# Leo-Liao-Chao/Uncertainty-Aware-CILQR-for-Trajectory-Optimization

Measured on AMD Instinct MI355X. Metric: CILQR solves/sec (N=50, batch B), higher is better.
Workload: dtype f64

## Files before the change

include/cilqr.h:

```cpp
#ifndef CILQR_H_
#define CILQR_H_

#include <stddef.h>
#include <stdint.h>

#ifdef __cplusplus
extern "C" {
#endif

#define CILQR_NX 4
#define CILQR_NU 2
#define CILQR_POLY_COEFFS 6
#define CILQR_MAX_HORIZON 384
#define CILQR_ABI_VERSION 2
#define CILQR_COMM_ID_BYTES 128
#define CILQR_MAX_POLYGONS 1024
#define CILQR_MAX_POLYGON_VERTICES 16

typedef struct cilqr_params {
  int32_t num_of_local_wpts;
  int32_t poly_order;
  int32_t horizon;
  int32_t max_iterations;
  int32_t num_states;
// ... 107 lines not shown
                                int32_t* iters_out, int32_t* status_out, uint32_t flags);
int cilqr_solve_batch_obstacles_device(cilqr_handle* h, void* stream, int B, int N, int M, const double* x0, double* U,
                                       const double* poly, const double* xplan_fl, const cilqr_obstacles* obs, double* X_out,
                                       double* J_out, int32_t* iters_out, int32_t* status_out, uint32_t flags);

int cilqr_set_uncertainty_map_device(cilqr_handle* h, const cilqr_uncertainty_map* map);
int cilqr_set_uncertainty_map(cilqr_handle* h, const cilqr_uncertainty_map* map);
int cilqr_clear_uncertainty_map(cilqr_handle* h);

int cilqr_debug_uncertainty_cost(cilqr_handle* h, int n, const double* states, double* cost, double* vx, double* mx);

int cilqr_solve_batch_sampled(cilqr_handle* h, int B, int N, int n_obs, int n_samples,
                              const double* x0, double* U, const double* poly, const double* xplan_fl,
                              const double* nom_pose, const double* nom_dim, const double* sample_offset,
                              double sample_weight, double* X_out, double* J_out, int32_t* iters_out,
                              int32_t* status_out, uint32_t flags);
int cilqr_solve_batch_sampled_device(cilqr_handle* h, void* stream, int B, int N, int n_obs, int n_samples,
                                     const double* x0, double* U, const double* poly, const double* xplan_fl,
                                     const double* nom_pose, const double* nom_dim, const double* sample_offset,
                                     double sample_weight, double* X_out, double* J_out, int32_t* iters_out,
                                     int32_t* status_out, uint32_t flags);

int cilqr_argmin_device(cilqr_handle* h, void* stream, int B, const double* J, double* out_pair);

#define CILQR_SCORE_FIELDS 8
typedef enum cilqr_score_field {
  CILQR_SCORE_TRACK = 0,
  CILQR_SCORE_CONTROL = 1,
  CILQR_SCORE_OBSTACLE = 2,
  CILQR_SCORE_UNCERTAINTY = 3,
  CILQR_SCORE_MAX_C = 4,
  CILQR_SCORE_MAX_C_ENTRY = 5,
  CILQR_SCORE_MAX_CTRL = 6,
  CILQR_SCORE_COLLISION = 7
} cilqr_score_field;
int cilqr_score_batch_device(cilqr_handle* h, void* stream, int B, int N, int M, const double* X, const double* U, const double* poly,
                             const double* xplan_fl, const cilqr_obstacles* obs, double max_collision, double* score, double* total);
int cilqr_score_batch(cilqr_handle* h, int B, int N, int M, const double* X, const double* U, const double* poly,
                      const double* xplan_fl, const cilqr_obstacles* obs, double max_collision, double* score, double* total);
int cilqr_score_batch_sampled_device(cilqr_handle* h, void* stream, int B, int N, int n_obs, int n_samples, const double* X,
                                     const double* U, const double* poly, const double* xplan_fl, const double* nom_pose,
                                     const double* nom_dim, const double* sample_offset, double sample_weight, double max_collision,
                                     double* score, double* total);
int cilqr_score_batch_sampled(cilqr_handle* h, int B, int N, int n_obs, int n_samples, const double* X, const double* U,
                              const double* poly, const double* xplan_fl, const double* nom_pose, const double* nom_dim,
                              const double* sample_offset, double sample_weight, double max_collision, double* score, double* total);
// ... 196 lines not shown
                              double max_risk, const double* base, double* risk, double* step_risk, double* pair_p, double* entry_p,
                              double* total);

int cilqr_predict_obstacles_device(cilqr_handle* h, void* stream, int T, int N, int M, const double* track, const double* track_dim,
                                   const double* track_cov, const double* track_noise, double* pose_out, double* dim_out,
                                   double* cov_out, double* sigma_out);
int cilqr_predict_obstacles(cilqr_handle* h, int T, int N, int M, const double* track, const double* track_dim, const double* track_cov,
                            const double* track_noise, double* pose_out, double* dim_out, double* cov_out, double* sigma_out);

int cilqr_chance_risk_cov_device(cilqr_handle* h, void* stream, int B, int N, int M, const double* X, const double* U, const double* K,
                                 const double* sigma0, int64_t sigma0_batch_stride, const double* process_noise,
                                 const cilqr_obstacles* obs, const double* obs_cov, uint32_t flags, double max_risk, const double* base,
                                 double* risk, double* step_risk, double* entry_p, double* sigma_out, double* total);
int cilqr_chance_risk_cov(cilqr_handle* h, int B, int N, int M, const double* X, const double* U, const double* K, const double* sigma0,
                          int64_t sigma0_batch_stride, const double* process_noise, const cilqr_obstacles* obs, const double* obs_cov,
                          uint32_t flags, double max_risk, const double* base, double* risk, double* step_risk, double* entry_p,
                          double* sigma_out, double* total);

int cilqr_comm_unique_id(void* id_bytes );
int cilqr_comm_init_rank(cilqr_handle* h, int n_ranks, int rank, const void* id_bytes);
int cilqr_comm_destroy(cilqr_handle* h);
int cilqr_comm_size(const cilqr_handle* h);
int cilqr_argmin_global_device(cilqr_handle* h, void* stream, int B, const double* J, int64_t index_offset, double* out_pair);

int cilqr_debug_select(cilqr_handle* h, int n, const double* triples, double* out_pair);

typedef struct cilqr_multi cilqr_multi;
int cilqr_create_multi(const cilqr_params* p, int max_batch_per_device, int max_horizon, int max_obstacles, int n_devices,
                       const int* devices, cilqr_multi** out);
int cilqr_multi_destroy(cilqr_multi* m);
int cilqr_multi_device_count(const cilqr_multi* m);
cilqr_handle* cilqr_multi_handle(cilqr_multi* m, int i);
int cilqr_shard_range(int B, int n_shards, int shard, int* first, int* count);
int cilqr_multi_solve_batch(cilqr_multi* m, int B, int N, int M, const double* x0, double* U, const double* poly,
                            const double* xplan_fl, const double* obs_pose, const double* obs_dim, const double* obs_weight,
                            double* X_out, double* J_out, int32_t* iters_out, int32_t* status_out, uint32_t flags,
                            int64_t* best_index, double* best_J);
int cilqr_multi_uses_rccl(const cilqr_multi* m);
int cilqr_debug_fail_enqueue(cilqr_handle* h, int nth_call);

int cilqr_set_diag_buffer(cilqr_handle* h, uint64_t* dev_buf);

int cilqr_set_pass_count_buffer(cilqr_handle* h, int32_t* dev_buf);

int cilqr_solve_family(const cilqr_handle* h, int B, int N, int M);
int cilqr_solve_wavefronts(const cilqr_handle* h, int B, int N, int M);
// ... 232 lines not shown
```

uncertainty-aware-cilqr-for-trajectory-optimization_amd/cilqr_amd/__init__.py:

```python
import ctypes as C
import os

import numpy as np

PKG_ROOT = os.path.dirname(os.path.dirname(os.path.abspath(__file__)))
LIB_PATH = os.environ.get("CILQR_LIB") or os.path.join(PKG_ROOT, "lib", "libcilqr_hip.so")

NX, NU, POLY = 4, 2, 6
FLAG_FAITHFUL_ITERS = 1
FLAG_GENERAL_ONLY = 2
EXIT_TOLERANCE, EXIT_LAMBDA_MAX, EXIT_MAX_ITER, EXIT_NUMERIC = 0, 1, 2, 3
SCORE_FIELDS = 8
(SCORE_TRACK, SCORE_CONTROL, SCORE_OBSTACLE, SCORE_UNCERTAINTY, SCORE_MAX_C, SCORE_MAX_C_ENTRY, SCORE_MAX_CTRL,
 SCORE_COLLISION) = range(SCORE_FIELDS)
RISK_FIELDS = 4
RISK_COLLISION, RISK_WORST_C, RISK_WORST_ROW, RISK_MEAN_TOTAL = range(RISK_FIELDS)
ROLLOUT_RISK_FIELDS = 6
RR_COLLISION, RR_WORST_C, RR_WORST_ROW, RR_WORST_ENTRY, RR_FIRST_STEP, RR_STEP_SHARE = range(ROLLOUT_RISK_FIELDS)
RRS_FIELDS = 8
(RRS_COLLISION, RRS_WORST_C, RRS_WORST_ROW, RRS_WORST_ENTRY, RRS_FIRST_STEP, RRS_STEP_SHARE, RRS_ANY_SHARE,
 RRS_PAIR_SHARE) = range(RRS_FIELDS)
MAP_RISK_FIELDS = 7
MR_COLLISION, MR_WORST_OCC, MR_WORST_ROW, MR_WORST_ENTRY, MR_FIRST_STEP, MR_STEP_SHARE, MR_UNKNOWN = range(MAP_RISK_FIELDS)
MAP_RISK_UNKNOWN_HITS = 1
# ... 35 lines not shown
TS_X, TS_Y, TS_VX, TS_VY, TS_P = 0, 1, 2, 3, 4
TS_SIZE_X, TS_SIZE_Y, TS_YAW, TS_ID, TS_HITS, TS_MISSES, TS_AGE, TS_DET = range(20, 28)
TRACK_WORLD_FIELDS = 9
(TW_NEXT_ID, TW_TICKS, TW_LIVE, TW_CONFIRMED, TW_MATCHED, TW_BORN, TW_DIED, TW_DROPPED,
 TW_INVALID) = range(TRACK_WORLD_FIELDS)
TRACK_RESET = 1
CLEAR_MOVERS_FIELDS = 8
(CM_MOVERS, CM_CLEARED, CM_OWNED_LINKED, CM_OWNED_HALO, CM_MAX_VALUE, CM_MAX_CELL, CM_CONTESTED,
 CM_KEPT_UNKNOWN) = range(CLEAR_MOVERS_FIELDS)
CLEAR_MOVERS_MAX_HALO2 = 1024
MAP_CLEARANCE_FIELDS = 8
(MC_CLEARANCE, MC_STEP, MC_CELL, MC_BELOW_STEPS, MC_FIRST_BELOW, MC_TOUCH_STEPS, MC_OFF_MAP_STEPS,
 MC_LOST_STEPS) = range(MAP_CLEARANCE_FIELDS)
MAP_CLEARANCE_UNKNOWN_SEEDS = 1
STOP_FIELDS = 8
(SP_STOP_STEP, SP_DISTANCE, SP_END_SPEED, SP_DEVIATION, SP_DEVIATION_STEP, SP_CLAMPED_STEPS, SP_OVERRUN_STEPS,
 SP_LOST) = range(STOP_FIELDS)
STOP_ALLOW_MOVING = 1
STOP_MIN_ADVANCE = 1.0e-3

ABI_SYMBOLS = (
    "cilqr_params_default", "cilqr_abi_version", "cilqr_device_count", "cilqr_last_error", "cilqr_default_control_seq",
    "cilqr_local_plan", "cilqr_local_plan_batch", "cilqr_local_plan_batch_device", "cilqr_create", "cilqr_destroy", "cilqr_host_alloc", "cilqr_host_free", "cilqr_solve_batch", "cilqr_solve_batch_device", "cilqr_solve_batch_obstacles", "cilqr_solve_batch_obstacles_device", "cilqr_solve_batch_sampled", "cilqr_solve_batch_sampled_device",
    "cilqr_argmin_device", "cilqr_wait", "cilqr_set_diag_buffer", "cilqr_set_pass_count_buffer", "cilqr_solve_family", "cilqr_solve_wavefronts", "cilqr_solve_sampled_wavefronts", "cilqr_debug_quu_inverse", "cilqr_debug_closest_sample", "cilqr_debug_blur_ellipse", "cilqr_warp_costmap", "cilqr_warp_costmap_device", "cilqr_warp_costmap_batch_device", "cilqr_blur_costmap", "cilqr_blur_costmap_device", "cilqr_blur_costmap_batch_device", "cilqr_map_geom_set",
    "cilqr_occupancy_to_layer", "cilqr_occupancy_to_layer_device", "cilqr_layer_to_occupancy", "cilqr_layer_to_occupancy_device",
    "cilqr_costmap_frame_device", "cilqr_costmap_frame_batch_device",
    "cilqr_boxes_to_polygons", "cilqr_rasterize_polygons", "cilqr_rasterize_polygons_device", "cilqr_warp_costmap_polygons_device",
    "cilqr_costmap_frame_polygons_device",
    "cilqr_set_uncertainty_map", "cilqr_set_uncertainty_map_device", "cilqr_clear_uncertainty_map", "cilqr_debug_uncertainty_cost",
    "cilqr_comm_unique_id", "cilqr_comm_init_rank", "cilqr_comm_destroy", "cilqr_comm_size", "cilqr_argmin_global_device", "cilqr_debug_select",
    "cilqr_create_multi", "cilqr_multi_destroy", "cilqr_multi_device_count", "cilqr_multi_handle", "cilqr_multi_solve_batch",
    "cilqr_shard_range", "cilqr_multi_uses_rccl", "cilqr_debug_fail_enqueue",
    "cilqr_score_batch", "cilqr_score_batch_device", "cilqr_score_batch_sampled", "cilqr_score_batch_sampled_device",
    "cilqr_gains_batch", "cilqr_gains_batch_device", "cilqr_rollout_batch", "cilqr_rollout_batch_device",
    "cilqr_score_rollouts", "cilqr_score_rollouts_device",
    "cilqr_rollout_risk", "cilqr_rollout_risk_device",
    "cilqr_gains_batch_sampled", "cilqr_gains_batch_sampled_device", "cilqr_rollout_risk_sampled", "cilqr_rollout_risk_sampled_device",
    "cilqr_rollout_risk_map", "cilqr_rollout_risk_map_device",
    "cilqr_chance_risk", "cilqr_chance_risk_device",
    "cilqr_tighten_obstacles", "cilqr_tighten_obstacles_device", "cilqr_chance_kappa",
    "cilqr_tighten_map", "cilqr_tighten_map_device",
    "cilqr_rasterize_tracks", "cilqr_rasterize_tracks_device",
    "cilqr_chance_risk_map", "cilqr_chance_risk_map_device", "cilqr_pose_quadrature",
    "cilqr_chance_risk_sampled", "cilqr_chance_risk_sampled_device",
    "cilqr_predict_obstacles", "cilqr_predict_obstacles_device", "cilqr_chance_risk_cov", "cilqr_chance_risk_cov_device",
    "cilqr_footprint_check", "cilqr_footprint_check_device",
    "cilqr_map_distance", "cilqr_map_distance_device", "cilqr_inflate_map", "cilqr_inflate_map_device",
    "cilqr_map_obstacles", "cilqr_map_obstacles_device",
    "cilqr_track_update", "cilqr_track_update_device",
    "cilqr_clear_movers", "cilqr_clear_movers_device",
    "cilqr_map_clearance", "cilqr_map_clearance_device",
    "cilqr_stop_plans", "cilqr_stop_plans_device",
)
# ... 1039 lines not shown
        if path.ndim == 3:
            if path.shape[0] != B:
                raise CilqrError("local_plan_batch: path batch dimension does not match ego")
            P, stride = path.shape[1], 2 * path.shape[1]
        else:
            path = path.reshape(-1, 2)
            P, stride = path.shape[0], 0
        W = self.params.num_of_local_wpts
        poly = np.zeros((B, POLY))
        fl = np.zeros((B, 2))
        ref = np.zeros((B, W, 2))
        n = np.zeros(B, dtype=np.int32)
        _check(lib().cilqr_local_plan_batch(self._h, B, int(P), _p(path), C.c_int64(stride), _p(ego), _p(poly), _p(fl), _p(ref),
                                            _p(n, _ip)))
        return dict(poly=poly, xplan_fl=fl, ref_traj=ref, n=n)

    def local_plan_batch_device(self, stream, B, P, path, path_stride, ego, poly, xplan_fl, ref_traj=0, n_out=0):
        _check(lib().cilqr_local_plan_batch_device(self._h, _vp(stream), int(B), int(P), _vp(path), C.c_int64(path_stride), _vp(ego),
                                                   _vp(poly), _vp(xplan_fl), _vp(ref_traj), _vp(n_out)))

    def argmin_device(self, stream, B, J, out_pair):
        _check(lib().cilqr_argmin_device(self._h, _vp(stream), int(B), _vp(J), _vp(out_pair)))

    def set_uncertainty_map(self, layer, geom, pose=(0.0, 0.0, 0.0), probes=(3, 3)):
        flat = np.ascontiguousarray(np.asfortranarray(layer, dtype=np.float32).flatten(order="F"))
        assert flat.size == geom.rows * geom.cols
        m = UncertaintyMap()
        m.layer = flat.ctypes.data
        m.geom = geom
        m.pose_x, m.pose_y, m.pose_theta = pose
        m.probes_l, m.probes_w = probes
        _check(lib().cilqr_set_uncertainty_map(self._h, C.byref(m)))

    def set_uncertainty_map_device(self, layer_ptr, geom, pose=(0.0, 0.0, 0.0), probes=(3, 3), layer_stride=0, poses_ptr=0):
        m = UncertaintyMap()
        m.layer = int(layer_ptr)
        m.geom = geom
        m.pose_x, m.pose_y, m.pose_theta = pose
        m.poses = int(poses_ptr) if poses_ptr else None
        m.layer_stride = int(layer_stride)
        m.probes_l, m.probes_w = probes
        _check(lib().cilqr_set_uncertainty_map_device(self._h, C.byref(m)))

    def clear_uncertainty_map(self):
        _check(lib().cilqr_clear_uncertainty_map(self._h))

    def debug_uncertainty_cost(self, states):
        states = _np64(states).reshape(-1, 4)
        n = states.shape[0]
        cost, vx, mx = np.zeros(n), np.zeros((n, 2)), np.zeros((n, 3))
        _check(lib().cilqr_debug_uncertainty_cost(self._h, n, _p(states), _p(cost), _p(vx), _p(mx)))
        return cost, vx, mx

    def comm_init_rank(self, n_ranks, rank, id_bytes):
        buf = (C.c_char * COMM_ID_BYTES).from_buffer_copy(bytes(id_bytes))
        _check(lib().cilqr_comm_init_rank(self._h, int(n_ranks), int(rank), buf))

    def comm_size(self):
        return int(lib().cilqr_comm_size(self._h))

    def argmin_global_device(self, stream, B, J, index_offset, out_pair):
        _check(lib().cilqr_argmin_global_device(self._h, _vp(stream), int(B), _vp(J), C.c_int64(index_offset), _vp(out_pair)))

    def debug_select(self, triples):
        t = _np64(triples).reshape(-1, 3)
        out = np.zeros(2)
        _check(lib().cilqr_debug_select(self._h, int(t.shape[0]), _p(t), _p(out)))
        return float(out[0]), int(out[1])

    def set_diag_buffer(self, dev_ptr):
        _check(lib().cilqr_set_diag_buffer(self._h, _vp(dev_ptr)))

    def set_pass_count_buffer(self, dev_ptr):
        _check(lib().cilqr_set_pass_count_buffer(self._h, _vp(dev_ptr)))

    def solve_family(self, B, N, M):
        g = lib().cilqr_solve_family(self._h, int(B), int(N), int(M))
        if g < 0:
            _check(g)
        return g

    def solve_wavefronts(self, B, N, M):
        w = lib().cilqr_solve_wavefronts(self._h, int(B), int(N), int(M))
        if w < 0:
            _check(w)
# ... 141 lines not shown
```

uncertainty-aware-cilqr-for-trajectory-optimization_amd/cilqr_amd/dist.py:

```python
import torch

_offset_cache = {}


def init_comm(solver, dist, group=None):
    world, rank = dist.get_world_size(group), dist.get_rank(group)
    from . import comm_unique_id
    box = [comm_unique_id() if rank == 0 else None]
    dist.broadcast_object_list(box, src=0, group=group)
    solver.comm_init_rank(world, rank, box[0])
    return world


def select_min_cost_device(solver, stream, B, J_ptr, index_offset, pair):
    solver.argmin_global_device(stream, B, J_ptr, index_offset, pair.data_ptr())
    j, i = pair.tolist()
    return j, int(i)


def select_min_cost(pair, index_offset, dist=None, group=None):
    if dist is None or not dist.is_initialized() or dist.get_world_size(group) == 1:
        j, i = pair.tolist()
        return j, (int(i) + index_offset if i >= 0 else int(i))
    world = dist.get_world_size(group)
    key = (str(pair.device), pair.dtype, int(index_offset))
    if key not in _offset_cache:
        _offset_cache[key] = torch.tensor([float(index_offset)], dtype=pair.dtype, device=pair.device)
    mine = torch.cat([pair.reshape(2), _offset_cache[key]])
    allp = torch.empty(world, 3, dtype=mine.dtype, device=mine.device)
    dist.all_gather_into_tensor(allp, mine.reshape(1, 3), group=group)
    rows = [(j, i + off if i >= 0 else i) for j, i, off in allp.tolist()]
    best = None
    for j, i in rows:
        if i < 0 or j != j:
            continue
        if best is None or j < best[0] or (j == best[0] and i < best[1]):
            best = (j, int(i))
    return best if best is not None else (float("inf"), -1)
```

uncertainty-aware-cilqr-for-trajectory-optimization_amd/csrc/cilqr_api.cpp:

```cpp
#include <math.h>
#include <stdarg.h>
#include <stdio.h>
#include <stdlib.h>
#include <string.h>

#include <new>
#include <string>
#include <vector>

#include "cilqr_internal.h"

#include "cilqr_handle.h"
#include "costmap_components.hpp"
#include "costmap_movers.hpp"

namespace cilqr {
thread_local std::string g_last_error;

int fail(int code, const char* fmt, ...) {
  char buf[512];
  va_list ap;
  va_start(ap, fmt);
  vsnprintf(buf, sizeof(buf), fmt, ap);
  va_end(ap);
// ... 205 lines not shown

  cilqr_handle* h = new (std::nothrow) cilqr_handle();
  if (!h) return fail(CILQR_ERR_ARG, "out of host memory");
  memset(h, 0, sizeof(*h));
  h->params = *p;
  derive(*p, h->kp);
  h->device = device;
  h->knobs = read_knobs(prop.multiProcessorCount > 0 ? prop.multiProcessorCount * 4 : 1024);
  h->max_batch = max_batch; h->max_horizon = max_horizon; h->max_obstacles = max_obstacles;
  const size_t B = max_batch, N = max_horizon, M = max_obstacles;
  hipError_t err = hipStreamCreateWithFlags(&h->stream, hipStreamNonBlocking);
  h->arena_cap = cilqr::host_arena_bytes(B, N, M);
  if (err == hipSuccess) err = hipMalloc((void**)&h->d_arena, h->arena_cap);
  h->stage_cap = h->arena_cap < ((size_t)1 << 20) ? h->arena_cap : ((size_t)1 << 20);
  if (err == hipSuccess) err = hipHostMalloc((void**)&h->stage, h->stage_cap, hipHostMallocDefault);
  const size_t Bpad = (B + 63) / 64 * 64;
  if (err == hipSuccess) err = dmalloc(&h->d_obs_tab, Bpad * M * N * 6);
  if (err == hipSuccess) err = dmalloc(&h->d_ws, cilqr::solve_groups_ws_doubles(max_batch, max_horizon));
  if (err == hipSuccess) err = dmalloc(&h->d_redo, B);
  if (err == hipSuccess) err = dmalloc(&h->d_hint_passes, B);
  if (err == hipSuccess) err = dmalloc(&h->d_order, B);
  h->hint_B = 0; h->hint_stream = nullptr;
  if (err == hipSuccess) err = dmalloc(&h->d_pair, (size_t)2);
  h->risk_part_stride = cilqr::RISK_PART_DOUBLES + (N + 1) / 2;
  if (err == hipSuccess) err = dmalloc(&h->d_risk_part, B * h->risk_part_stride);
  if (err == hipSuccess) err = dmalloc(&h->d_chance_map_steps, 3 * B * N);
  if (err == hipSuccess) err = dmalloc(&h->d_chance_sampled_steps, cilqr::CHANCE_SAMPLED_REC * B * N);
  if (err == hipSuccess) err = dmalloc(&h->d_footprint_steps, cilqr::footprint_scratch_doubles(B, N));
  if (err == hipSuccess) err = dmalloc(&h->d_tighten_map_part, (size_t)cilqr::TIGHTEN_MAP_REC * cilqr::TIGHTEN_MAP_MAX_G * B);
  if (err == hipSuccess) err = dmalloc(&h->d_track_map_rec, (size_t)cilqr::TRACK_MAP_ENTRY * B * M * N);
  if (err == hipSuccess) err = dmalloc(&h->d_track_map_part, (size_t)cilqr::TRACK_MAP_REC * cilqr::TRACK_MAP_MAX_G * B);
  if (err == hipSuccess) err = dmalloc(&h->d_triple, (size_t)3);
  if (err == hipSuccess) err = dmalloc(&h->d_gather, (size_t)3);
  h->comm_ranks = 1;
  if (err == hipSuccess) err = dmalloc(&h->d_oob, (size_t)1);
  if (err == hipSuccess) err = dmalloc(&h->d_poses, (size_t)8 * 1024 * 4);
  if (err == hipSuccess) err = dmalloc(&h->d_polys, (size_t)8 * cilqr::POLYGON_TABLE_DOUBLES);
  if (err == hipSuccess) err = dmalloc(&h->d_occ_steps, (size_t)8 * 128);
  if (err == hipSuccess) {
    void* unused = nullptr;
    const size_t W = (size_t)p->num_of_local_wpts;
    if (cilqr::scratch_bytes(h, cilqr::SCR_PLAN_IO, (B * (4 + CILQR_POLY_COEFFS + 2 + 2 * W)) * sizeof(double) + B * sizeof(int32_t), &unused) != CILQR_OK ||
        cilqr::scratch_bytes(h, cilqr::SCR_PLAN_PATH, 2 * 1024 * sizeof(double), &unused) != CILQR_OK)
      err = hipErrorOutOfMemory;
  }
  if (err != hipSuccess) {
    int rc = fail(CILQR_ERR_HIP, "cilqr_create: device allocation failed: %s", hipGetErrorString(err));
    cilqr_destroy(h);
    return rc;
  }
  *out = h;
  return CILQR_OK;
}

int cilqr_destroy(cilqr_handle* h) {
  if (!h) return CILQR_OK;
  (void)hipSetDevice(h->device);
  if (h->stream) (void)hipStreamSynchronize(h->stream);
  (void)cilqr_comm_destroy(h);
  if (h->stage) (void)hipHostFree(h->stage);
  for (void* p : h->scratch)
    if (p) (void)hipFree(p);
  void* ptrs[] = {h->d_poses, h->d_polys, h->d_unc_layer, h->d_triple, h->d_gather, h->d_arena, h->d_obs_tab, h->d_ws, h->d_redo, h->d_hint_passes, h->d_order, h->d_pair, h->d_risk_part, h->d_chance_map_steps, h->d_chance_sampled_steps, h->d_footprint_steps, h->d_tighten_map_part, h->d_track_map_rec, h->d_track_map_part, h->d_src, h->d_dst, h->d_bbox, h->d_oob, h->d_occ_steps};
  for (void* p : ptrs)
    if (p) (void)hipFree(p);
  if (h->stream) (void)hipStreamDestroy(h->stream);
  delete h;
  return CILQR_OK;
}

int cilqr_set_diag_buffer(cilqr_handle* h, uint64_t* dev_buf) {
  if (!h) return fail(CILQR_ERR_ARG, "null handle");
  h->diag = (unsigned long long*)dev_buf;
  return CILQR_OK;
}

namespace {
int fill_unc(const cilqr_handle* h, const cilqr_uncertainty_map* m, cilqr::UncArgs& u) {
  if (!m || !m->layer) return fail(CILQR_ERR_ARG, "cilqr_set_uncertainty_map: null map or layer");
  const cilqr_map_geom& g = m->geom;
  if (g.rows < 2 || g.cols < 2 || !(g.res > 0.0) || !(g.len_x > 0.0) || !(g.len_y > 0.0))
    return fail(CILQR_ERR_ARG, "cilqr_set_uncertainty_map: bad geometry (needs at least 2x2 cells)");
  if (m->probes_l < 1 || m->probes_w < 1 || m->probes_l > 64 || m->probes_w > 64)
// ... 251 lines not shown
                              const double* sample_offset, double sample_weight, double* X_out, double* J_out,
                              int32_t* iters_out, int32_t* status_out, uint32_t flags) {
  int rc = check_sampled(h, "cilqr_solve_batch_sampled", B, N, n_obs, n_samples);
  if (rc) return rc;
  if (B == 0) return CILQR_OK;
  if (!x0 || !U || !poly || !xplan_fl || !X_out || !nom_pose || !nom_dim || !sample_offset)
    return fail(CILQR_ERR_ARG, "cilqr_solve_batch_sampled: null required pointer");
  cilqr_obstacles o{nom_pose, nom_dim, nullptr, 0, 0, 0, 0};
  cilqr::HostPlan p(h->d_arena);
  cilqr::plan_solve(p, B, N, n_obs, n_samples, x0, U, poly, xplan_fl, o, (size_t)B * n_obs * N, 0, sample_offset, X_out, J_out, iters_out, status_out);
  return cilqr::host_call(h, p, [&] {
    const int rc = cilqr_solve_batch_sampled_device(h, h->stream, B, N, n_obs, n_samples, x0, U, poly, xplan_fl, o.pose, o.dim, sample_offset,
                                                    sample_weight, X_out, J_out, iters_out, status_out, flags);
    if (rc == CILQR_OK) h->d_J = J_out;
    return rc;
  }, true);
}

int cilqr_argmin_device(cilqr_handle* h, void* stream, int B, const double* J, double* out_pair) {
  if (!h || !J || !out_pair || B < 1) return fail(CILQR_ERR_ARG, "cilqr_argmin_device: bad argument");
  HIP_TRY(hipSetDevice(h->device));
  HIP_TRY(cilqr::launch_argmin(J, B, out_pair, nullptr, 0.0, (hipStream_t)stream));
  return CILQR_OK;
}

namespace {
int score_device(cilqr_handle* h, void* stream, cilqr::ScoreArgs& a, const double* X, const double* U, const double* poly,
                 const double* xplan_fl, double max_collision, double* score, double* total, int n_counters) {
  cilqr::SolveArgs& s = a.s;
  s.X_out = const_cast<double*>(X);
  s.U = const_cast<double*>(U);
  s.poly = poly; s.xplan_fl = xplan_fl;
  a.score = score; a.total = total; a.max_collision = max_collision; a.w_uncertainty = h->params.w_uncertainty;
  if (a.rows < 1) a.rows = 1;
  if (cilqr::score_lds_bytes(s.N, h->kp.n_samples, n_counters) > cilqr::SCORE_LDS_MAX)
    return fail(CILQR_ERR_UNSUPPORTED, "cilqr_score_batch: %d path samples, horizon %d and %d sample counters do not fit 64 KiB of LDS",
                h->kp.n_samples, s.N, n_counters);
  HIP_TRY(hipSetDevice(h->device));
  HIP_TRY(cilqr::launch_score(a, (hipStream_t)stream));
  return CILQR_OK;
}
}

int cilqr_score_batch_device(cilqr_handle* h, void* stream, int B, int N, int M, const double* X, const double* U, const double* poly,
                             const double* xplan_fl, const cilqr_obstacles* obs, double max_collision, double* score, double* total) {
  int rc = check_sizes(h, B, N, M);
// ... 1987 lines not shown
```

uncertainty-aware-cilqr-for-trajectory-optimization_amd/csrc/cilqr_comm.cpp:

```cpp
#include <rccl/rccl.h>

#include <math.h>
#include <string.h>

#include <new>
#include <set>
#include <string>
#include <thread>
#include <vector>

#include "cilqr_handle.h"

using cilqr::fail;

#define NCCL_TRY(expr)                                                                                      \
  do {                                                                                                      \
    ncclResult_t r_ = (expr);                                                                               \
    if (r_ != ncclSuccess) return fail(CILQR_ERR_COMM, "%s failed: %s", #expr, ncclGetErrorString(r_));     \
  } while (0)

static_assert(CILQR_COMM_ID_BYTES == NCCL_UNIQUE_ID_BYTES, "cilqr.h carries RCCL's unique id verbatim");

struct cilqr_multi {
  std::vector<cilqr_handle*> h;
  std::vector<int> devices;
  int max_batch_per_device;
  bool rccl;
  std::vector<hipEvent_t> ev;
};

namespace {

int set_gather(cilqr_handle* h, int n_ranks) {
  HIP_TRY(hipSetDevice(h->device));
  if (h->d_gather) (void)hipFree(h->d_gather);
  h->d_gather = nullptr;
  HIP_TRY(hipMalloc((void**)&h->d_gather, sizeof(double) * 3 * (size_t)n_ranks));
  return CILQR_OK;
}

}

extern "C" {

int cilqr_shard_range(int B, int n_shards, int shard, int* first, int* count) {
  if (B < 0 || n_shards < 1 || shard < 0 || shard >= n_shards || !first || !count) return fail(CILQR_ERR_ARG, "cilqr_shard_range: bad argument");
  const int base = B / n_shards, rem = B % n_shards;
  *first = shard * base + (shard < rem ? shard : rem);
  *count = base + (shard < rem ? 1 : 0);
  return CILQR_OK;
}

int cilqr_comm_unique_id(void* id_bytes) {
  if (!id_bytes) return fail(CILQR_ERR_ARG, "cilqr_comm_unique_id: null argument");
  ncclUniqueId id;
  NCCL_TRY(ncclGetUniqueId(&id));
  memcpy(id_bytes, id.internal, NCCL_UNIQUE_ID_BYTES);
  return CILQR_OK;
}

// ... 10 lines not shown
  h->comm = c;
  h->comm_ranks = n_ranks;
  h->comm_rank = rank;
  return CILQR_OK;
}

int cilqr_comm_destroy(cilqr_handle* h) {
  if (!h) return fail(CILQR_ERR_ARG, "null handle");
  if (h->comm) {
    (void)hipSetDevice(h->device);
    ncclResult_t r = ncclCommDestroy(h->comm);
    h->comm = nullptr;
    h->comm_ranks = 1;
    h->comm_rank = 0;
    if (r != ncclSuccess) return fail(CILQR_ERR_COMM, "ncclCommDestroy failed: %s", ncclGetErrorString(r));
  }
  return CILQR_OK;
}

int cilqr_comm_size(const cilqr_handle* h) { return h ? (h->comm ? h->comm_ranks : 1) : 0; }

int cilqr_argmin_global_device(cilqr_handle* h, void* stream, int B, const double* J, int64_t index_offset, double* out_pair) {
  if (!h || !out_pair || B < 0 || (B > 0 && !J) || index_offset < 0) return fail(CILQR_ERR_ARG, "cilqr_argmin_global_device: bad argument");
  HIP_TRY(hipSetDevice(h->device));
  hipStream_t s = (hipStream_t)stream;
  if (!h->comm && B > 0) {
    HIP_TRY(cilqr::launch_argmin(J, B, out_pair, nullptr, 0.0, s, (double)index_offset));
    return CILQR_OK;
  }
  if (B > 0) {
    HIP_TRY(cilqr::launch_argmin(J, B, nullptr, h->d_triple, (double)index_offset, s));
  } else {
    const double none[3] = {HUGE_VAL, -1.0, 0.0};
    HIP_TRY(hipMemcpyAsync(h->d_triple, none, sizeof(none), hipMemcpyHostToDevice, s));
  }
  const double* gathered = h->d_triple;
  int n = 1;
  if (h->comm) {
    NCCL_TRY(ncclAllGather(h->d_triple, h->d_gather, 3, ncclDouble, h->comm, s));
    gathered = h->d_gather;
    n = h->comm_ranks;
  }
  HIP_TRY(cilqr::launch_select(gathered, n, out_pair, s));
  return CILQR_OK;
}

int cilqr_debug_select(cilqr_handle* h, int n, const double* triples, double* out_pair) {
  if (!h || n < 1 || !triples || !out_pair) return fail(CILQR_ERR_ARG, "cilqr_debug_select: bad argument");
  HIP_TRY(hipSetDevice(h->device));
  void* v = nullptr;
  int rc = cilqr::scratch_bytes(h, cilqr::SCR_DEBUG, sizeof(double) * 3 * (size_t)n, &v);
  if (rc) return rc;
  double* d = (double*)v;
  HIP_TRY(hipMemcpyAsync(d, triples, sizeof(double) * 3 * (size_t)n, hipMemcpyHostToDevice, h->stream));
  HIP_TRY(cilqr::launch_select(d, n, h->d_pair, h->stream));
  HIP_TRY(hipMemcpyAsync(out_pair, h->d_pair, sizeof(double) * 2, hipMemcpyDeviceToHost, h->stream));
  HIP_TRY(hipStreamSynchronize(h->stream));
  return CILQR_OK;
}

int cilqr_create_multi(const cilqr_params* p, int max_batch_per_device, int max_horizon, int max_obstacles, int n_devices,
                       const int* devices, cilqr_multi** out) {
  if (!p || !out || n_devices < 1) return fail(CILQR_ERR_ARG, "cilqr_create_multi: bad argument");
  *out = nullptr;
  int count = 0;
  if (hipGetDeviceCount(&count) != hipSuccess || count <= 0)
    return fail(CILQR_ERR_NO_DEVICE, "no HIP device available; this library has no CPU path");
// ... 126 lines not shown
    if (rcs[d]) return multi_abort(m, rcs[d], msgs[d]);
  if (m->rccl) {
    ncclResult_t r = ncclGroupStart();
    for (int d = 0; d < n && r == ncclSuccess; ++d) {
      cilqr_handle* h = m->h[d];
      r = ncclAllGather(h->d_triple, h->d_gather, 3, ncclDouble, h->comm, h->stream);
    }
    const ncclResult_t r_end = ncclGroupEnd();
    if (r == ncclSuccess) r = r_end;
    if (r != ncclSuccess) return multi_abort(m, CILQR_ERR_COMM, std::string("RCCL all-gather failed: ") + ncclGetErrorString(r));
  } else {
    cilqr_handle* h0 = m->h[0];
    hipError_t e = hipSetDevice(h0->device);
    for (int d = 0; d < n && e == hipSuccess; ++d) {
      e = hipStreamWaitEvent(h0->stream, m->ev[d], 0);
      if (e == hipSuccess) e = hipMemcpyAsync(h0->d_gather + 3 * (size_t)d, m->h[d]->d_triple, 3 * sizeof(double), hipMemcpyDeviceToDevice, h0->stream);
    }
    if (e != hipSuccess) return multi_abort(m, CILQR_ERR_HIP, std::string("record gather failed: ") + hipGetErrorString(e));
  }
  double pair[2] = {HUGE_VAL, -1.0};
  {
    cilqr_handle* h = m->h[0];
    hipError_t e = hipSetDevice(h->device);
    if (e == hipSuccess) e = cilqr::launch_select(h->d_gather, n, h->d_pair, h->stream);
    if (e == hipSuccess) e = hipMemcpyAsync(pair, h->d_pair, sizeof(pair), hipMemcpyDeviceToHost, h->stream);
    if (e != hipSuccess) return multi_abort(m, CILQR_ERR_HIP, std::string("min-cost pick failed: ") + hipGetErrorString(e));
  }
  for (int d = 0; d < n; ++d) {
    int rc = cilqr::host_finish(m->h[d]);
    if (rc == CILQR_OK && hipStreamSynchronize(m->h[d]->stream) != hipSuccess) rc = fail(CILQR_ERR_HIP, "hipStreamSynchronize failed");
    if (rc) return multi_abort(m, rc, cilqr::g_last_error);
  }
  if (best_J) *best_J = pair[0];
  if (best_index) *best_index = (int64_t)pair[1];
  return CILQR_OK;
}

}
```

uncertainty-aware-cilqr-for-trajectory-optimization_amd/csrc/cilqr_handle.h:

```cpp
#pragma once

#include <string>

#include "cilqr_host_plan.h"
#include "cilqr_internal.h"

struct ncclComm;

struct cilqr_handle;

namespace cilqr {
struct PendingOut {
  bool active, packed;
  int n;
  HostPlan::Entry out[HostPlan::CAP];
};
int host_copy_in(cilqr_handle* h, const HostPlan& p, bool solve);
int host_copy_out(cilqr_handle* h, const HostPlan& p, int launch_rc);
int host_finish(cilqr_handle* h);
template <typename Launch>
int host_enqueue(cilqr_handle* h, const HostPlan& p, Launch&& launch, bool solve = false) {
  const int rc = host_copy_in(h, p, solve);
  return rc ? rc : host_copy_out(h, p, launch());
}
// ... 22 lines not shown
  cilqr_params params;
  cilqr::KParams kp;
  int device;
  cilqr::SolveKnobs knobs;
  int max_batch, max_horizon, max_obstacles;
  hipStream_t stream;
  char* d_arena;
  size_t arena_cap;
  char* stage;
  size_t stage_cap;
  cilqr::PendingOut pending;
  int debug_fail_enqueue;
  double* d_J;
  void* scratch[cilqr::SCR_SLOTS];
  size_t scratch_cap[cilqr::SCR_SLOTS];
  double* d_obs_tab;
  double* d_ws;
  int32_t* d_redo;
  int32_t* d_hint_passes;
  int32_t* d_order;
  int hint_B;
  void* hint_stream;
  double* d_pair;
  double* d_risk_part;
  size_t risk_part_stride;
  double* d_chance_map_steps;
  double* d_tighten_map_part;
  double* d_track_map_rec;
  double* d_track_map_part;
  double* d_footprint_steps;
  double* d_chance_sampled_steps;
  float *d_src, *d_dst, *d_bbox;
  size_t src_cap, dst_cap, bbox_cap;
  unsigned long long* d_oob;
  double* d_poses;
  unsigned pose_slot;
  double* d_polys;
  unsigned poly_slot;
  float* d_occ_steps;
  unsigned occ_slot;
  unsigned long long* diag;
  int32_t* passes;
  cilqr::UncArgs unc;
  double unc_res;
  float* d_unc_layer;
  size_t unc_layer_cap;
  ncclComm* comm;
  int comm_ranks, comm_rank;
  double* d_triple;
  double* d_gather;
};
```

uncertainty-aware-cilqr-for-trajectory-optimization_amd/csrc/cilqr_internal.h:

```cpp
#pragma once

#include <hip/hip_runtime.h>
#include <stdint.h>

#include "cilqr.h"
#include "cilqr_wave_plan.h"

namespace cilqr {

struct KParams {
  double dt;
  double desired_speed;
  double tolerance;
  double w_acc, w_yawrate, w_pos, w_vel, w_obstacle;
  double q1_acc, q2_acc, q1_yawrate, q2_yawrate;
  double q1_front, q2_front, q1_rear, q2_rear;
  double acc_max, acc_min;
  double yaw_hi, yaw_lo;
  double half_dt2;
  double wheelbase, speed_max;
  double t_safe, s_safe_a, s_safe_b, ego_rad, ego_front, ego_rear;
  double lamb_factor, lamb_max;
  int32_t max_iterations;
  int32_t n_samples;
// ... 402 lines not shown
  double max_deviation, decel_weight;
  int32_t B, N, D, hold;
  int32_t plans;
  uint32_t flags;
  double dt, half_dt2, acc_max, acc_min, yaw_hi, yaw_lo, speed_max;
};
int stop_plans_per_group(int N, int D);
hipError_t launch_stop_plans(const StopArgs& a, hipStream_t stream);

struct LocalPlanArgs {
  const double* path;
  long long path_stride;
  const double* ego;
  double* poly;
  double* xplan_fl;
  double* ref_traj;
  int32_t* n_out;
  int32_t B, P, n_wpts, cols;
};
hipError_t launch_local_plan(const LocalPlanArgs& a, hipStream_t stream);
size_t local_plan_lds_bytes(int n_wpts, int cols);

hipError_t launch_argmin(const double* J, int B, double* out_pair, double* out_triple, double offset, hipStream_t stream,
                         double pair_offset = 0.0);
hipError_t launch_select(const double* triples, int n_ranks, double* out_pair, hipStream_t stream);

struct WarpArgs {
  const float* src;
  float* dst;
  const float* bbox;
  unsigned long long* n_oob;
  cilqr_map_geom sg, dg;
  double vx, vy, sin_t, cos_t;
};
hipError_t launch_warp(const WarpArgs& a, hipStream_t stream);
struct WarpBatchArgs {
  const float* src;
  float* dst;
  const float* bbox;
  unsigned long long* n_oob;
  const double* poses;
  double pose0[4];
  cilqr_map_geom sg, dg;
};
hipError_t launch_warp_batch(const WarpBatchArgs& a, int K, hipStream_t stream);

struct PolygonTable {
  const double* table;
// ... 34 lines not shown
```

uncertainty-aware-cilqr-for-trajectory-optimization_amd/csrc/cilqr_select.hip:

```cpp
#include "cilqr_internal.h"

namespace cilqr {

namespace {

constexpr int AM_THREADS = 1024;

__device__ __forceinline__ void amin_merge(double& j0, long long& i0, double j1, long long i1) {
  if (j1 < j0 || (j1 == j0 && i1 < i0)) { j0 = j1; i0 = i1; }
}

__global__ __launch_bounds__(AM_THREADS) void argmin_kernel(const double* J, int B, double* out_pair, double* out_triple, double offset,
                                                            double pair_offset) {
  __shared__ double sj[AM_THREADS / 64];
  __shared__ long long si[AM_THREADS / 64];
  constexpr long long NONE = 0x7fffffffffffffffll;
  double bj = __builtin_huge_val();
  long long bi = NONE;
  for (int i = threadIdx.x; i < B; i += AM_THREADS) amin_merge(bj, bi, J[i], i);
  for (int o = 32; o > 0; o >>= 1) {
    const double oj = __shfl_xor(bj, o, 64);
    const long long oi = __shfl_xor(bi, o, 64);
    amin_merge(bj, bi, oj, oi);
  }
  const int lane = threadIdx.x & 63, wave = threadIdx.x >> 6;
  if (lane == 0) { sj[wave] = bj; si[wave] = bi; }
  __syncthreads();
  if (threadIdx.x == 0) {
    for (int w = 1; w < AM_THREADS / 64; ++w) amin_merge(bj, bi, sj[w], si[w]);
    const double idx = (bi == NONE) ? -1.0 : (double)bi;
    if (out_pair) { out_pair[0] = bj; out_pair[1] = idx < 0.0 ? idx : idx + pair_offset; }
    if (out_triple) { out_triple[0] = bj; out_triple[1] = idx; out_triple[2] = offset; }
  }
}

__global__ __launch_bounds__(64) void select_kernel(const double* triples, int n_ranks, double* out_pair) {
  constexpr long long NONE = 0x7fffffffffffffffll;
  double bj = __builtin_huge_val();
  long long bi = NONE;
  for (int r = threadIdx.x; r < n_ranks; r += 64) {
    const double j = triples[3 * r], idx = triples[3 * r + 1], off = triples[3 * r + 2];
    if (idx >= 0.0) amin_merge(bj, bi, j, (long long)idx + (long long)off);
  }
  for (int o = 32; o > 0; o >>= 1) {
    const double oj = __shfl_xor(bj, o, 64);
    const long long oi = __shfl_xor(bi, o, 64);
    amin_merge(bj, bi, oj, oi);
  }
  if (threadIdx.x == 0) {
    out_pair[0] = bj;
    out_pair[1] = (bi == NONE) ? -1.0 : (double)bi;
  }
}

}

hipError_t launch_argmin(const double* J, int B, double* out_pair, double* out_triple, double offset, hipStream_t stream,
                         double pair_offset) {
  hipLaunchKernelGGL(argmin_kernel, dim3(1), dim3(AM_THREADS), 0, stream, J, B, out_pair, out_triple, offset, pair_offset);
  return hipGetLastError();
}

hipError_t launch_select(const double* triples, int n_ranks, double* out_pair, hipStream_t stream) {
  hipLaunchKernelGGL(select_kernel, dim3(1), dim3(64), 0, stream, triples, n_ranks, out_pair);
  return hipGetLastError();
}

}
```

Baseline: 2.598 million.

## Write min-cost pick to mapped host memory and use single-wave argmin for small batches

The argmin and select kernels can now write their result directly into a coherent, mapped pinned host buffer, fenced with a system-scope fence. Host callers sync the stream and read that buffer instead of issuing a separate device-to-host copy or a torch tolist. A single-wavefront argmin kernel with unrolled loads replaces the 1024-thread block when B is 4096 or less. Together these aim to cut per-pick launch, copy and sync latency, at the cost of extra API surface and reliance on coherent host-mapped writes.

```diff
diff --git a/include/cilqr.h b/include/cilqr.h
--- a/include/cilqr.h
+++ b/include/cilqr.h
@@ -153,6 +153,7 @@
                                      int32_t* status_out, uint32_t flags);
 
 int cilqr_argmin_device(cilqr_handle* h, void* stream, int B, const double* J, double* out_pair);
+int cilqr_argmin_device_read(cilqr_handle* h, void* stream, int B, const double* J, double* out_pair, double host_pair[2]);
 
 #define CILQR_SCORE_FIELDS 8
 typedef enum cilqr_score_field {
@@ -395,6 +396,8 @@
 int cilqr_comm_destroy(cilqr_handle* h);
 int cilqr_comm_size(const cilqr_handle* h);
 int cilqr_argmin_global_device(cilqr_handle* h, void* stream, int B, const double* J, int64_t index_offset, double* out_pair);
+int cilqr_argmin_global_device_read(cilqr_handle* h, void* stream, int B, const double* J, int64_t index_offset, double* out_pair,
+                                    double host_pair[2]);
 
 int cilqr_debug_select(cilqr_handle* h, int n, const double* triples, double* out_pair);
 
diff --git a/uncertainty-aware-cilqr-for-trajectory-optimization_amd/cilqr_amd/__init__.py b/uncertainty-aware-cilqr-for-trajectory-optimization_amd/cilqr_amd/__init__.py
--- a/uncertainty-aware-cilqr-for-trajectory-optimization_amd/cilqr_amd/__init__.py
+++ b/uncertainty-aware-cilqr-for-trajectory-optimization_amd/cilqr_amd/__init__.py
@@ -81,13 +81,13 @@
 ABI_SYMBOLS = (
     "cilqr_params_default", "cilqr_abi_version", "cilqr_device_count", "cilqr_last_error", "cilqr_default_control_seq",
     "cilqr_local_plan", "cilqr_local_plan_batch", "cilqr_local_plan_batch_device", "cilqr_create", "cilqr_destroy", "cilqr_host_alloc", "cilqr_host_free", "cilqr_solve_batch", "cilqr_solve_batch_device", "cilqr_solve_batch_obstacles", "cilqr_solve_batch_obstacles_device", "cilqr_solve_batch_sampled", "cilqr_solve_batch_sampled_device",
-    "cilqr_argmin_device", "cilqr_wait", "cilqr_set_diag_buffer", "cilqr_set_pass_count_buffer", "cilqr_solve_family", "cilqr_solve_wavefronts", "cilqr_solve_sampled_wavefronts", "cilqr_debug_quu_inverse", "cilqr_debug_closest_sample", "cilqr_debug_blur_ellipse", "cilqr_warp_costmap", "cilqr_warp_costmap_device", "cilqr_warp_costmap_batch_device", "cilqr_blur_costmap", "cilqr_blur_costmap_device", "cilqr_blur_costmap_batch_device", "cilqr_map_geom_set",
+    "cilqr_argmin_device", "cilqr_argmin_device_read", "cilqr_wait", "cilqr_set_diag_buffer", "cilqr_set_pass_count_buffer", "cilqr_solve_family", "cilqr_solve_wavefronts", "cilqr_solve_sampled_wavefronts", "cilqr_debug_quu_inverse", "cilqr_debug_closest_sample", "cilqr_debug_blur_ellipse", "cilqr_warp_costmap", "cilqr_warp_costmap_device", "cilqr_warp_costmap_batch_device", "cilqr_blur_costmap", "cilqr_blur_costmap_device", "cilqr_blur_costmap_batch_device", "cilqr_map_geom_set",
     "cilqr_occupancy_to_layer", "cilqr_occupancy_to_layer_device", "cilqr_layer_to_occupancy", "cilqr_layer_to_occupancy_device",
     "cilqr_costmap_frame_device", "cilqr_costmap_frame_batch_device",
     "cilqr_boxes_to_polygons", "cilqr_rasterize_polygons", "cilqr_rasterize_polygons_device", "cilqr_warp_costmap_polygons_device",
     "cilqr_costmap_frame_polygons_device",
     "cilqr_set_uncertainty_map", "cilqr_set_uncertainty_map_device", "cilqr_clear_uncertainty_map", "cilqr_debug_uncertainty_cost",
-    "cilqr_comm_unique_id", "cilqr_comm_init_rank", "cilqr_comm_destroy", "cilqr_comm_size", "cilqr_argmin_global_device", "cilqr_debug_select",
+    "cilqr_comm_unique_id", "cilqr_comm_init_rank", "cilqr_comm_destroy", "cilqr_comm_size", "cilqr_argmin_global_device", "cilqr_argmin_global_device_read", "cilqr_debug_select",
     "cilqr_create_multi", "cilqr_multi_destroy", "cilqr_multi_device_count", "cilqr_multi_handle", "cilqr_multi_solve_batch",
     "cilqr_shard_range", "cilqr_multi_uses_rccl", "cilqr_debug_fail_enqueue",
     "cilqr_score_batch", "cilqr_score_batch_device", "cilqr_score_batch_sampled", "cilqr_score_batch_sampled_device",
@@ -1173,6 +1173,11 @@
     def argmin_device(self, stream, B, J, out_pair):
         _check(lib().cilqr_argmin_device(self._h, _vp(stream), int(B), _vp(J), _vp(out_pair)))
 
+    def argmin_device_read(self, stream, B, J, out_pair=0):
+        host = (C.c_double * 2)()
+        _check(lib().cilqr_argmin_device_read(self._h, _vp(stream), int(B), _vp(J), _vp(out_pair), host))
+        return host[0], int(host[1])
+
     def set_uncertainty_map(self, layer, geom, pose=(0.0, 0.0, 0.0), probes=(3, 3)):
         flat = np.ascontiguousarray(np.asfortranarray(layer, dtype=np.float32).flatten(order="F"))
         assert flat.size == geom.rows * geom.cols
@@ -1212,6 +1217,11 @@
 
     def argmin_global_device(self, stream, B, J, index_offset, out_pair):
         _check(lib().cilqr_argmin_global_device(self._h, _vp(stream), int(B), _vp(J), C.c_int64(index_offset), _vp(out_pair)))
+
+    def argmin_global_device_read(self, stream, B, J, index_offset, out_pair=0):
+        host = (C.c_double * 2)()
+        _check(lib().cilqr_argmin_global_device_read(self._h, _vp(stream), int(B), _vp(J), C.c_int64(index_offset), _vp(out_pair), host))
+        return host[0], int(host[1])
 
     def debug_select(self, triples):
         t = _np64(triples).reshape(-1, 3)
diff --git a/uncertainty-aware-cilqr-for-trajectory-optimization_amd/cilqr_amd/dist.py b/uncertainty-aware-cilqr-for-trajectory-optimization_amd/cilqr_amd/dist.py
--- a/uncertainty-aware-cilqr-for-trajectory-optimization_amd/cilqr_amd/dist.py
+++ b/uncertainty-aware-cilqr-for-trajectory-optimization_amd/cilqr_amd/dist.py
@@ -1,4 +1,8 @@
+import os
+
 import torch
+
+PICK_BY_COPY = os.environ.get("CILQR_PICK_COPY", "0") == "1"
 
 _offset_cache = {}
 
@@ -13,9 +17,11 @@
 
 
 def select_min_cost_device(solver, stream, B, J_ptr, index_offset, pair):
-    solver.argmin_global_device(stream, B, J_ptr, index_offset, pair.data_ptr())
-    j, i = pair.tolist()
-    return j, int(i)
+    if PICK_BY_COPY:
+        solver.argmin_global_device(stream, B, J_ptr, index_offset, pair.data_ptr())
+        j, i = pair.tolist()
+        return j, int(i)
+    return solver.argmin_global_device_read(stream, B, J_ptr, index_offset, pair.data_ptr() if pair is not None else 0)
 
 
 def select_min_cost(pair, index_offset, dist=None, group=None):
diff --git a/uncertainty-aware-cilqr-for-trajectory-optimization_amd/csrc/cilqr_api.cpp b/uncertainty-aware-cilqr-for-trajectory-optimization_amd/csrc/cilqr_api.cpp
--- a/uncertainty-aware-cilqr-for-trajectory-optimization_amd/csrc/cilqr_api.cpp
+++ b/uncertainty-aware-cilqr-for-trajectory-optimization_amd/csrc/cilqr_api.cpp
@@ -251,6 +251,8 @@
   if (err == hipSuccess) err = dmalloc(&h->d_order, B);
   h->hint_B = 0; h->hint_stream = nullptr;
   if (err == hipSuccess) err = dmalloc(&h->d_pair, (size_t)2);
+  if (err == hipSuccess) err = hipHostMalloc((void**)&h->pick_host, 2 * sizeof(double), hipHostMallocCoherent | hipHostMallocMapped);
+  if (err == hipSuccess) err = hipHostGetDevicePointer((void**)&h->pick_dev, h->pick_host, 0);
   h->risk_part_stride = cilqr::RISK_PART_DOUBLES + (N + 1) / 2;
   if (err == hipSuccess) err = dmalloc(&h->d_risk_part, B * h->risk_part_stride);
   if (err == hipSuccess) err = dmalloc(&h->d_chance_map_steps, 3 * B * N);
@@ -288,6 +290,7 @@
   if (h->stream) (void)hipStreamSynchronize(h->stream);
   (void)cilqr_comm_destroy(h);
   if (h->stage) (void)hipHostFree(h->stage);
+  if (h->pick_host) (void)hipHostFree(h->pick_host);
   for (void* p : h->scratch)
     if (p) (void)hipFree(p);
   void* ptrs[] = {h->d_poses, h->d_polys, h->d_unc_layer, h->d_triple, h->d_gather, h->d_arena, h->d_obs_tab, h->d_ws, h->d_redo, h->d_hint_passes, h->d_order, h->d_pair, h->d_risk_part, h->d_chance_map_steps, h->d_chance_sampled_steps, h->d_footprint_steps, h->d_tighten_map_part, h->d_track_map_rec, h->d_track_map_part, h->d_src, h->d_dst, h->d_bbox, h->d_oob, h->d_occ_steps};
@@ -585,6 +588,13 @@
   HIP_TRY(hipSetDevice(h->device));
   HIP_TRY(cilqr::launch_argmin(J, B, out_pair, nullptr, 0.0, (hipStream_t)stream));
   return CILQR_OK;
+}
+
+int cilqr_argmin_device_read(cilqr_handle* h, void* stream, int B, const double* J, double* out_pair, double host_pair[2]) {
+  if (!h || !J || !host_pair || B < 1) return fail(CILQR_ERR_ARG, "cilqr_argmin_device_read: bad argument");
+  HIP_TRY(hipSetDevice(h->device));
+  HIP_TRY(cilqr::launch_argmin(J, B, out_pair, nullptr, 0.0, (hipStream_t)stream, 0.0, h->pick_dev));
+  return cilqr::read_pick(h, (hipStream_t)stream, host_pair);
 }
 
 namespace {
diff --git a/uncertainty-aware-cilqr-for-trajectory-optimization_amd/csrc/cilqr_comm.cpp b/uncertainty-aware-cilqr-for-trajectory-optimization_amd/csrc/cilqr_comm.cpp
--- a/uncertainty-aware-cilqr-for-trajectory-optimization_amd/csrc/cilqr_comm.cpp
+++ b/uncertainty-aware-cilqr-for-trajectory-optimization_amd/csrc/cilqr_comm.cpp
@@ -36,6 +36,29 @@
   if (h->d_gather) (void)hipFree(h->d_gather);
   h->d_gather = nullptr;
   HIP_TRY(hipMalloc((void**)&h->d_gather, sizeof(double) * 3 * (size_t)n_ranks));
+  return CILQR_OK;
+}
+
+int enqueue_global_pick(cilqr_handle* h, hipStream_t s, int B, const double* J, int64_t index_offset, double* out_pair, double* host_slot) {
+  HIP_TRY(hipSetDevice(h->device));
+  if (!h->comm && B > 0) {
+    HIP_TRY(cilqr::launch_argmin(J, B, out_pair, nullptr, 0.0, s, (double)index_offset, host_slot));
+    return CILQR_OK;
+  }
+  if (B > 0) {
+    HIP_TRY(cilqr::launch_argmin(J, B, nullptr, h->d_triple, (double)index_offset, s));
+  } else {
+    const double none[3] = {HUGE_VAL, -1.0, 0.0};
+    HIP_TRY(hipMemcpyAsync(h->d_triple, none, sizeof(none), hipMemcpyHostToDevice, s));
+  }
+  const double* gathered = h->d_triple;
+  int n = 1;
+  if (h->comm) {
+    NCCL_TRY(ncclAllGather(h->d_triple, h->d_gather, 3, ncclDouble, h->comm, s));
+    gathered = h->d_gather;
+    n = h->comm_ranks;
+  }
+  HIP_TRY(cilqr::launch_select(gathered, n, out_pair, s, host_slot));
   return CILQR_OK;
 }
 
@@ -92,27 +115,14 @@
 
 int cilqr_argmin_global_device(cilqr_handle* h, void* stream, int B, const double* J, int64_t index_offset, double* out_pair) {
   if (!h || !out_pair || B < 0 || (B > 0 && !J) || index_offset < 0) return fail(CILQR_ERR_ARG, "cilqr_argmin_global_device: bad argument");
-  HIP_TRY(hipSetDevice(h->device));
-  hipStream_t s = (hipStream_t)stream;
-  if (!h->comm && B > 0) {
-    HIP_TRY(cilqr::launch_argmin(J, B, out_pair, nullptr, 0.0, s, (double)index_offset));
-    return CILQR_OK;
-  }
-  if (B > 0) {
-    HIP_TRY(cilqr::launch_argmin(J, B, nullptr, h->d_triple, (double)index_offset, s));
-  } else {
-    const double none[3] = {HUGE_VAL, -1.0, 0.0};
-    HIP_TRY(hipMemcpyAsync(h->d_triple, none, sizeof(none), hipMemcpyHostToDevice, s));
-  }
-  const double* gathered = h->d_triple;
-  int n = 1;
-  if (h->comm) {
-    NCCL_TRY(ncclAllGather(h->d_triple, h->d_gather, 3, ncclDouble, h->comm, s));
-    gathered = h->d_gather;
-    n = h->comm_ranks;
-  }
-  HIP_TRY(cilqr::launch_select(gathered, n, out_pair, s));
-  return CILQR_OK;
+  return enqueue_global_pick(h, (hipStream_t)stream, B, J, index_offset, out_pair, nullptr);
+}
+
+int cilqr_argmin_global_device_read(cilqr_handle* h, void* stream, int B, const double* J, int64_t index_offset, double* out_pair,
+                                    double host_pair[2]) {
+  if (!h || !host_pair || B < 0 || (B > 0 && !J) || index_offset < 0) return fail(CILQR_ERR_ARG, "cilqr_argmin_global_device_read: bad argument");
+  const int rc = enqueue_global_pick(h, (hipStream_t)stream, B, J, index_offset, out_pair, h->pick_dev);
+  return rc ? rc : cilqr::read_pick(h, (hipStream_t)stream, host_pair);
 }
 
 int cilqr_debug_select(cilqr_handle* h, int n, const double* triples, double* out_pair) {
@@ -285,8 +295,7 @@
   {
     cilqr_handle* h = m->h[0];
     hipError_t e = hipSetDevice(h->device);
-    if (e == hipSuccess) e = cilqr::launch_select(h->d_gather, n, h->d_pair, h->stream);
-    if (e == hipSuccess) e = hipMemcpyAsync(pair, h->d_pair, sizeof(pair), hipMemcpyDeviceToHost, h->stream);
+    if (e == hipSuccess) e = cilqr::launch_select(h->d_gather, n, nullptr, h->stream, h->pick_dev);
     if (e != hipSuccess) return multi_abort(m, CILQR_ERR_HIP, std::string("min-cost pick failed: ") + hipGetErrorString(e));
   }
   for (int d = 0; d < n; ++d) {
@@ -294,6 +303,11 @@
     if (rc == CILQR_OK && hipStreamSynchronize(m->h[d]->stream) != hipSuccess) rc = fail(CILQR_ERR_HIP, "hipStreamSynchronize failed");
     if (rc) return multi_abort(m, rc, cilqr::g_last_error);
   }
+  {
+    const volatile double* slot = m->h[0]->pick_host;
+    pair[0] = slot[0];
+    pair[1] = slot[1];
+  }
   if (best_J) *best_J = pair[0];
   if (best_index) *best_index = (int64_t)pair[1];
   return CILQR_OK;
diff --git a/uncertainty-aware-cilqr-for-trajectory-optimization_amd/csrc/cilqr_handle.h b/uncertainty-aware-cilqr-for-trajectory-optimization_amd/csrc/cilqr_handle.h
--- a/uncertainty-aware-cilqr-for-trajectory-optimization_amd/csrc/cilqr_handle.h
+++ b/uncertainty-aware-cilqr-for-trajectory-optimization_amd/csrc/cilqr_handle.h
@@ -68,6 +68,8 @@
   int hint_B;
   void* hint_stream;
   double* d_pair;
+  double* pick_host;
+  double* pick_dev;
   double* d_risk_part;
   size_t risk_part_stride;
   double* d_chance_map_steps;
@@ -96,3 +98,13 @@
   double* d_triple;
   double* d_gather;
 };
+
+namespace cilqr {
+inline int read_pick(cilqr_handle* h, hipStream_t stream, double host_pair[2]) {
+  HIP_TRY(hipStreamSynchronize(stream));
+  const volatile double* slot = h->pick_host;
+  host_pair[0] = slot[0];
+  host_pair[1] = slot[1];
+  return CILQR_OK;
+}
+}
diff --git a/uncertainty-aware-cilqr-for-trajectory-optimization_amd/csrc/cilqr_internal.h b/uncertainty-aware-cilqr-for-trajectory-optimization_amd/csrc/cilqr_internal.h
--- a/uncertainty-aware-cilqr-for-trajectory-optimization_amd/csrc/cilqr_internal.h
+++ b/uncertainty-aware-cilqr-for-trajectory-optimization_amd/csrc/cilqr_internal.h
@@ -448,8 +448,8 @@
 size_t local_plan_lds_bytes(int n_wpts, int cols);
 
 hipError_t launch_argmin(const double* J, int B, double* out_pair, double* out_triple, double offset, hipStream_t stream,
-                         double pair_offset = 0.0);
-hipError_t launch_select(const double* triples, int n_ranks, double* out_pair, hipStream_t stream);
+                         double pair_offset = 0.0, double* host_pair = nullptr);
+hipError_t launch_select(const double* triples, int n_ranks, double* out_pair, hipStream_t stream, double* host_pair = nullptr);
 
 struct WarpArgs {
   const float* src;
diff --git a/uncertainty-aware-cilqr-for-trajectory-optimization_amd/csrc/cilqr_select.hip b/uncertainty-aware-cilqr-for-trajectory-optimization_amd/csrc/cilqr_select.hip
--- a/uncertainty-aware-cilqr-for-trajectory-optimization_amd/csrc/cilqr_select.hip
+++ b/uncertainty-aware-cilqr-for-trajectory-optimization_amd/csrc/cilqr_select.hip
@@ -10,8 +10,21 @@
   if (j1 < j0 || (j1 == j0 && i1 < i0)) { j0 = j1; i0 = i1; }
 }
 
+__device__ __forceinline__ void store_pick(double* out_pair, double* host_pair, double j, double idx) {
+  if (out_pair) { out_pair[0] = j; out_pair[1] = idx; }
+  if (host_pair) { host_pair[0] = j; host_pair[1] = idx; __threadfence_system(); }
+}
+
+__device__ __forceinline__ void argmin_write(double bj, long long bi, double* out_pair, double* out_triple, double offset, double pair_offset,
+                                             double* host_pair) {
+  constexpr long long NONE = 0x7fffffffffffffffll;
+  const double idx = (bi == NONE) ? -1.0 : (double)bi;
+  if (out_triple) { out_triple[0] = bj; out_triple[1] = idx; out_triple[2] = offset; }
+  store_pick(out_pair, host_pair, bj, idx < 0.0 ? idx : idx + pair_offset);
+}
+
 __global__ __launch_bounds__(AM_THREADS) void argmin_kernel(const double* J, int B, double* out_pair, double* out_triple, double offset,
-                                                            double pair_offset) {
+                                                            double pair_offset, double* host_pair) {
   __shared__ double sj[AM_THREADS / 64];
   __shared__ long long si[AM_THREADS / 64];
   constexpr long long NONE = 0x7fffffffffffffffll;
@@ -28,13 +41,36 @@
   __syncthreads();
   if (threadIdx.x == 0) {
     for (int w = 1; w < AM_THREADS / 64; ++w) amin_merge(bj, bi, sj[w], si[w]);
-    const double idx = (bi == NONE) ? -1.0 : (double)bi;
-    if (out_pair) { out_pair[0] = bj; out_pair[1] = idx < 0.0 ? idx : idx + pair_offset; }
-    if (out_triple) { out_triple[0] = bj; out_triple[1] = idx; out_triple[2] = offset; }
+    argmin_write(bj, bi, out_pair, out_triple, offset, pair_offset, host_pair);
   }
 }
 
-__global__ __launch_bounds__(64) void select_kernel(const double* triples, int n_ranks, double* out_pair) {
+constexpr int AM_WAVE_MAX = 4096;
+constexpr int AM_WAVE_UNROLL = 8;
+__global__ __launch_bounds__(64) void argmin_wave_kernel(const double* J, int B, double* out_pair, double* out_triple, double offset,
+                                                         double pair_offset, double* host_pair) {
+  constexpr long long NONE = 0x7fffffffffffffffll;
+  double bj = __builtin_huge_val();
+  long long bi = NONE;
+  for (int base = threadIdx.x; base < B; base += 64 * AM_WAVE_UNROLL) {
+    double v[AM_WAVE_UNROLL];
+#pragma unroll
+    for (int k = 0; k < AM_WAVE_UNROLL; ++k) {
+      const int i = base + 64 * k;
+      v[k] = i < B ? J[i] : __builtin_nan("");
+    }
+#pragma unroll
+    for (int k = 0; k < AM_WAVE_UNROLL; ++k) amin_merge(bj, bi, v[k], base + 64 * k);
+  }
+  for (int o = 32; o > 0; o >>= 1) {
+    const double oj = __shfl_xor(bj, o, 64);
+    const long long oi = __shfl_xor(bi, o, 64);
+    amin_merge(bj, bi, oj, oi);
+  }
+  if (threadIdx.x == 0) argmin_write(bj, bi, out_pair, out_triple, offset, pair_offset, host_pair);
+}
+
+__global__ __launch_bounds__(64) void select_kernel(const double* triples, int n_ranks, double* out_pair, double* host_pair) {
   constexpr long long NONE = 0x7fffffffffffffffll;
   double bj = __builtin_huge_val();
   long long bi = NONE;
@@ -47,22 +83,22 @@
     const long long oi = __shfl_xor(bi, o, 64);
     amin_merge(bj, bi, oj, oi);
   }
-  if (threadIdx.x == 0) {
-    out_pair[0] = bj;
-    out_pair[1] = (bi == NONE) ? -1.0 : (double)bi;
-  }
+  if (threadIdx.x == 0) store_pick(out_pair, host_pair, bj, (bi == NONE) ? -1.0 : (double)bi);
 }
 
 }
 
 hipError_t launch_argmin(const double* J, int B, double* out_pair, double* out_triple, double offset, hipStream_t stream,
-                         double pair_offset) {
-  hipLaunchKernelGGL(argmin_kernel, dim3(1), dim3(AM_THREADS), 0, stream, J, B, out_pair, out_triple, offset, pair_offset);
+                         double pair_offset, double* host_pair) {
+  if (B <= AM_WAVE_MAX)
+    hipLaunchKernelGGL(argmin_wave_kernel, dim3(1), dim3(64), 0, stream, J, B, out_pair, out_triple, offset, pair_offset, host_pair);
+  else
+    hipLaunchKernelGGL(argmin_kernel, dim3(1), dim3(AM_THREADS), 0, stream, J, B, out_pair, out_triple, offset, pair_offset, host_pair);
   return hipGetLastError();
 }
 
-hipError_t launch_select(const double* triples, int n_ranks, double* out_pair, hipStream_t stream) {
-  hipLaunchKernelGGL(select_kernel, dim3(1), dim3(64), 0, stream, triples, n_ranks, out_pair);
+hipError_t launch_select(const double* triples, int n_ranks, double* out_pair, hipStream_t stream, double* host_pair) {
+  hipLaunchKernelGGL(select_kernel, dim3(1), dim3(64), 0, stream, triples, n_ranks, out_pair, host_pair);
   return hipGetLastError();
 }
 
```

Measured after the change: 2.615 million (median of 6 runs). Within noise of the previous version (+0.6%).
